# formeo/igaming-platform

Measured on AMD Instinct MI355X. Metric: fraud scores/sec (whole node) + p99 score latency, higher is better.
Workload: dtype fp32

## Files before the change

### csrc/runtime/bindings.cpp

```cpp
#include <pybind11/numpy.h>
#include <pybind11/pybind11.h>
#include <pybind11/stl.h>

#include <atomic>
#include <cstring>
#include <memory>
#include <thread>

#include "account_index.h"
#include "acct_core.h"
#include "acct_devices.h"
#include "audit.h"
#include "h2grpc.h"
#include "cpu_device.h"
#include "cpu_scorer.h"
#include "serve_core.h"
#include "link_index.h"
#include "mult_sketch.h"
#include "executor.h"
#include "onnx_model.h"
#include "sampler.h"
#include "trees.h"
#include "wire.h"
#include "xxh64.h"
// ... 526 lines not shown
        load("ring_ts", c.ring_ts.data(), c.ring_ts.size() * 4);
        load("ring_amt", c.ring_amt.data(), c.ring_amt.size() * 8);
        load("hll", c.hll.data(), c.hll.size());
        load("rt", c.rt.data(), c.rt.size() * sizeof(AcctRT));
        load("batch", c.batch.data(), c.batch.size() * sizeof(AcctBatch));
        load("ext", c.ext.data(), c.ext.size() * 4);
        load("ev", c.ev.data(), c.ev.size() * 2);
      })
      .def_property_readonly("capacity", &CpuScorer::capacity);

  auto view = [](py::array res, py::object feat, py::object ms, wire::ResultView& v,
                 py::array& keep_r, py::object& keep_f, py::object& keep_m) {
    keep_r = py::array_t<uint32_t, py::array::c_style | py::array::forcecast>(res);
    if (keep_r.ndim() != 2 || keep_r.shape(1) != 2) throw std::runtime_error("results must be [n,2] (ResultRec)");
    v.n = size_t(keep_r.shape(0));
    v.res = reinterpret_cast<const ResultRec*>(keep_r.data());
    v.feat = nullptr;
    v.response_ms = nullptr;
    if (!feat.is_none()) {
      auto f = py::array_t<int32_t, py::array::c_style | py::array::forcecast>(feat);
      if (f.ndim() != 2 || f.shape(1) != 32 || size_t(f.shape(0)) != v.n) throw std::runtime_error("features must be [n,32] (FeatRec)");
      keep_f = f;
      v.feat = reinterpret_cast<const FeatRec*>(f.data());
    }
    if (!ms.is_none()) {
      auto t = py::array_t<int64_t, py::array::c_style | py::array::forcecast>(ms);
      if (size_t(t.size()) != v.n) throw std::runtime_error("response_ms length mismatch");
      keep_m = t;
      v.response_ms = t.data();
    }
  };
  m.def("serialize_batch_response", [view](py::array res, py::object feat, py::object ms) {
    wire::ResultView v;
    py::array kr; py::object kf, km;
    view(res, feat, ms, v, kr, kf, km);
    std::string out;
    {
      py::gil_scoped_release rel;
      out = wire::serialize_batch_response(v);
    }
    return py::bytes(out);
  }, py::arg("results"), py::arg("features") = py::none(), py::arg("response_ms") = py::none());
  m.def("serialize_tx_response", [view](py::array res, py::object feat, py::object ms, size_t i) {
    wire::ResultView v;
    py::array kr; py::object kf, km;
    view(res, feat, ms, v, kr, kf, km);
    if (i >= v.n) throw std::runtime_error("index out of range");
    return py::bytes(wire::serialize_tx_response(v, i));
  }, py::arg("results"), py::arg("features") = py::none(), py::arg("response_ms") = py::none(), py::arg("index") = 0);
  m.def("serialize_tx_responses", [view](py::array res, py::object feat, py::object ms) {
    wire::ResultView v;
    py::array kr; py::object kf, km;
    view(res, feat, ms, v, kr, kf, km);
    std::vector<std::string> outs(v.n);
    {
      py::gil_scoped_release rel;
      for (size_t i = 0; i < v.n; ++i) outs[i] = wire::serialize_tx_response(v, i);
    }
    py::list l;
    for (auto& o : outs) l.append(py::bytes(o));
    return l;
  }, py::arg("results"), py::arg("features") = py::none(), py::arg("response_ms") = py::none());
  m.def("serialize_feature_vector", [](py::array feat) {
    auto f = py::array_t<int32_t, py::array::c_style | py::array::forcecast>(feat);
    if (f.size() != 32) throw std::runtime_error("FeatRec must have 32 int32 words");
    return py::bytes(wire::serialize_feature_vector(*reinterpret_cast<const FeatRec*>(f.data())));
  });

  py::class_<StepClock, std::shared_ptr<StepClock>>(m, "StepClock")
      .def(py::init<const std::string&, int, int, bool>(), py::arg("shm_name"), py::arg("world"), py::arg("rank"),
           py::arg("create"))
      .def(py::init<int>(), py::arg("world"))
      .def("issued", &StepClock::issued)
      .def("max_issued", &StepClock::max_issued)
      .def("hold_of", &StepClock::hold_of)
      .def("set_rank", &StepClock::set_rank)
      .def("unlink_shared", &StepClock::unlink_shared)
      .def_property_readonly("world", &StepClock::world)
      .def_property_readonly("rank", &StepClock::rank);

  py::class_<CpuDevice, std::shared_ptr<CpuDevice>>(m, "CpuDevice")
      .def(py::init<std::shared_ptr<CpuScorer>, int, int>(), py::arg("scorer"), py::arg("depth") = 2,
           py::arg("cap") = 8192, py::keep_alive<1, 2>())
      .def("device_ops", [](const CpuDevice& d) { return reinterpret_cast<uintptr_t>(d.ops()); });

  py::class_<ShmXchgDevice, std::shared_ptr<ShmXchgDevice>>(m, "ShmXchgDevice")
      .def(py::init<std::shared_ptr<CpuScorer>, const std::string&, int, int, int, int, bool, double>(),
           py::arg("scorer"), py::arg("shm_name"), py::arg("world"), py::arg("rank"), py::arg("depth"), py::arg("C"),
           py::arg("create"), py::arg("timeout_s") = 60.0, py::keep_alive<1, 2>())
      .def("device_ops", [](const ShmXchgDevice& d) { return reinterpret_cast<uintptr_t>(d.ops()); })
      .def_property_readonly("rows_scored", &ShmXchgDevice::rows_scored)
      .def_property_readonly("slot_violations", &ShmXchgDevice::slot_violations)
      .def_property_readonly("steps", &ShmXchgDevice::steps)
      .def("debug_stall_results_when", &ShmXchgDevice::debug_stall_results_when)
      .def("unlink_shared", &ShmXchgDevice::unlink_shared);

  py::class_<AuditRing, std::shared_ptr<AuditRing>>(m, "AuditRing")
      .def(py::init<int64_t>(), py::arg("capacity"))
      .def("pending", &AuditRing::pending)
      .def("append", [](AuditRing& a, py::array_t<uint32_t, py::array::c_style> res,
                        py::array_t<int32_t, py::array::c_style> slots, int owner, int64_t t_ms, int version) {
        const size_t n = size_t(slots.size());
        if (res.ndim() != 2 || size_t(res.shape(0)) != n || res.shape(1) != 2)
          throw std::runtime_error("AuditRing.append: res must be uint32[n,2] for n slots");
        const ResultRec* r = reinterpret_cast<const ResultRec*>(res.data());
        const int32_t* s = slots.data();
        py::gil_scoped_release rel;
        a.append(r, s, 1, owner, n, t_ms, uint16_t(version));
      }, py::arg("res"), py::arg("slots"), py::arg("owner"), py::arg("t_ms"), py::arg("version"))
      .def_property_readonly("evicted", &AuditRing::evicted)
      .def_property_readonly("appended", &AuditRing::appended)
      .def("flush_sqlite", [](AuditRing& a, const std::string& path, const std::string& schema,
                              std::vector<std::shared_ptr<AccountIndex>> idx) {
        py::gil_scoped_release rel;
        return a.flush_sqlite(path, schema, idx);
      })
      .def_property_readonly("capacity", &AuditRing::capacity)
      .def("flush_segment", [](AuditRing& a, const std::string& dir, const std::string& tag,
                               std::vector<std::shared_ptr<AccountIndex>> idx) {
        py::gil_scoped_release rel;
        return a.flush_segment(dir, tag, idx);
      })
      .def("peek", [](const AuditRing& a, int64_t max) {
        auto v = a.peek(max);
        py::dict d;
        std::vector<int64_t> t(v.size());
        std::vector<int32_t> sl(v.size()), ow(v.size()), ver(v.size());
        std::vector<uint32_t> pk(v.size());
        std::vector<float> ml(v.size());
        for (size_t i = 0; i < v.size(); ++i) {
          t[i] = v[i].t_ms; sl[i] = v[i].slot; ow[i] = v[i].owner; ver[i] = v[i].model_version;
          pk[i] = v[i].packed; ml[i] = v[i].ml;
        }
        d["t_ms"] = vec_np(t); d["slot"] = vec_np(sl); d["owner"] = vec_np(ow); d["model_version"] = vec_np(ver);
        d["packed"] = vec_np(pk); d["ml"] = vec_np(ml);
        return d;
      }, py::arg("max") = 1 << 20);

  m.def("audit_load_segment", [](const std::string& seg, const std::string& db, const std::string& schema) {
    py::gil_scoped_release rel;
    return audit_load_segment(seg, db, schema);
  }, py::arg("segment"), py::arg("db"), py::arg("schema"));

  py::class_<PyGrpc>(m, "GrpcServer")
      .def(py::init([](py::object core, py::function cold, int cold_threads, int batch_threads, py::object acct) {
             auto p = std::make_unique<PyGrpc>();
             std::shared_ptr<ServeCore> c;
             if (!core.is_none()) {
               c = core.cast<PyServe&>().core;
               p->core = core;
             }
             std::shared_ptr<AcctRouter> ar;
             if (!acct.is_none()) {
               ar = acct.cast<PyAcct&>().router;
               p->acct = acct;
             }
             GrpcServer::ColdFn fn = [cb = py::function(cold)](const std::string& path, std::string body) {
               py::gil_scoped_acquire g;
               GrpcReply r;
               try {
                 py::object out = cb(py::str(path), py::bytes(body));
                 if (py::isinstance<py::bytes>(out)) {
                   r.body = out.cast<std::string>();
                 } else {
                   auto t = out.cast<py::tuple>();
                   r.status = t[0].cast<int>();
                   r.message = t[1].cast<std::string>();
// ... 483 lines not shown
```

### csrc/runtime/cpu_device.cpp

```cpp
#include "cpu_device.h"

#include <unistd.h>

#include <chrono>
#include <cstring>
#include <stdexcept>
#include <thread>

namespace igp {
namespace {

void set_err(char* err, int32_t errlen, const char* msg) {
  if (!err || errlen <= 0) return;
  std::strncpy(err, msg, size_t(errlen) - 1);
  err[errlen - 1] = 0;
}

}

CpuDevice::CpuDevice(std::shared_ptr<CpuScorer> sc, int depth, int cap) : sc_(std::move(sc)) {
  if (!sc_ || depth < 1 || cap < 1) throw std::runtime_error("CpuDevice: scorer / depth / capacity");
  slots_.resize(depth);
  for (auto& s : slots_) {
    s.rows.resize(cap);
    s.res.resize(cap);
    s.feat.resize(cap);
  }
  ops_.abi = IGP_DEVICE_OPS_ABI;
  ops_.depth = depth;
  ops_.world = 1;
  ops_.exchange = 0;
  ops_.cap = cap;
  ops_.features_always = 0;
  ops_.ctx = this;
  ops_.rows = &rows_fn;
  ops_.submit = &submit_fn;
  ops_.wait = &wait_fn;
  ops_.results = &results_fn;
  ops_.features = &features_fn;
}

char* CpuDevice::rows_fn(void* ctx, int32_t slot) {
  return reinterpret_cast<char*>(static_cast<CpuDevice*>(ctx)->slots_[slot].rows.data());
}

int32_t CpuDevice::submit_fn(void* ctx, int32_t slot, int32_t n, int32_t, int64_t now, int32_t wf, char* err,
                             int32_t errlen) {
  auto* d = static_cast<CpuDevice*>(ctx);
  Slot& s = d->slots_[slot];
  try {
    s.wf = (wf & IGP_SUBMIT_WANT_FEATURES) != 0;
    d->sc_->score(s.rows.data(), size_t(n), now, true, s.res.data(), s.wf ? s.feat.data() : nullptr);
  } catch (const std::exception& e) {
    set_err(err, errlen, e.what());
    return -1;
  }
  return 0;
}

int32_t CpuDevice::wait_fn(void*, int32_t, int64_t, char*, int32_t) { return 0; }

const void* CpuDevice::results_fn(void* ctx, int32_t slot) {
  return static_cast<CpuDevice*>(ctx)->slots_[slot].res.data();
}

const void* CpuDevice::features_fn(void* ctx, int32_t slot) {
  const Slot& s = static_cast<CpuDevice*>(ctx)->slots_[slot];
  return s.wf ? s.feat.data() : nullptr;
}

ShmXchgDevice::ShmXchgDevice(std::shared_ptr<CpuScorer> sc, const std::string& shm_name, int world, int rank, int depth,
                             int C, bool create, double timeout_s)
    : sc_(std::move(sc)), world_(world), rank_(rank), C_(C), timeout_s_(timeout_s) {
  if (!sc_ || world < 1 || rank < 0 || rank >= world || depth < 1 || C < 1)
    throw std::runtime_error("ShmXchgDevice: bad arguments");
  W_ = sizeof(ResultRec) + sizeof(FeatRec);
  send_bytes_ = size_t(world) * size_t(C + 1) * sizeof(ReqRec);
  res_bytes_ = size_t(world) * size_t(C) * W_;
  const size_t flag_bytes = sizeof(int64_t) * OwnerGenerations::kLineWords * kRing * size_t(world);
  const size_t bytes = sizeof(Counter) * size_t(world) + flag_bytes + size_t(world) * kRing * (send_bytes_ + res_bytes_);
  region_ = Region::shared(shm_name, bytes, create);
  counters_ = reinterpret_cast<Counter*>(region_.base());
  char* flags = reinterpret_cast<char*>(region_.base()) + sizeof(Counter) * size_t(world);
  owners_ = OwnerGenerations(reinterpret_cast<int64_t*>(flags), world, rank);
  data_ = flags + flag_bytes;
  slots_.resize(depth);
  for (auto& s : slots_) {
    s.send.resize(size_t(world) * size_t(C + 1));
    s.recv.resize(res_bytes_);
  }
  compact_.resize(size_t(world) * size_t(C));
  route_.resize(size_t(world) * size_t(C));
  res_.resize(size_t(world) * size_t(C));
  feat_.resize(size_t(world) * size_t(C));
  ops_.abi = IGP_DEVICE_OPS_ABI;
  ops_.depth = depth;
  ops_.world = world;
  ops_.exchange = 1;
  ops_.cap = C;
  ops_.features_always = 1;
  ops_.ctx = this;
  ops_.rows = &rows_fn;
  ops_.submit = &submit_fn;
  ops_.wait = &wait_fn;
  ops_.results = &results_fn;
  ops_.features = &features_fn;
}

ReqRec* ShmXchgDevice::send_area(int r, int q) const {
  return reinterpret_cast<ReqRec*>(data_ + (size_t(r) * kRing + size_t(q)) * send_bytes_);
}

char* ShmXchgDevice::res_area(int r, int q) const {
  return data_ + size_t(world_) * kRing * send_bytes_ + (size_t(r) * kRing + size_t(q)) * res_bytes_;
}

void ShmXchgDevice::wait_all(std::atomic<int64_t> Counter::*field, int64_t target) {
  const auto t_end = std::chrono::steady_clock::now() + std::chrono::duration<double>(timeout_s_);
  for (int spin = 0;; ++spin) {
    bool all = true;
    for (int r = 0; r < world_ && all; ++r) all = (counters_[r].*field).load(std::memory_order_acquire) >= target;
    if (all) return;
    if (spin < 2000) {
      std::this_thread::yield();
    } else {
      if (std::chrono::steady_clock::now() > t_end) throw std::runtime_error("ShmXchgDevice: a peer missed the step");
      std::this_thread::sleep_for(std::chrono::microseconds(20));
    }
  }
}

void ShmXchgDevice::step(int slot, int64_t now) {
// ... 69 lines not shown
```

### csrc/runtime/cpu_device.h

```cpp
#pragma once
#include <atomic>
#include <memory>
#include <string>
#include <vector>

#include "../include/device_ops.h"
#include "../include/records.h"
#include "../include/results_region.h"
#include "cpu_scorer.h"
#include "shm.h"

namespace igp {

class CpuDevice {
 public:
  CpuDevice(std::shared_ptr<CpuScorer> sc, int depth, int cap);
  const IgpDeviceOps* ops() const { return &ops_; }

 private:
  struct Slot {
    std::vector<ReqRec> rows;
    std::vector<ResultRec> res;
    std::vector<FeatRec> feat;
    bool wf = false;
  };
  static char* rows_fn(void* ctx, int32_t slot);
  static int32_t submit_fn(void* ctx, int32_t slot, int32_t n, int32_t seq, int64_t now, int32_t wf, char* err, int32_t errlen);
  static int32_t wait_fn(void* ctx, int32_t slot, int64_t timeout_us, char* err, int32_t errlen);
  static const void* results_fn(void* ctx, int32_t slot);
  static const void* features_fn(void* ctx, int32_t slot);
  std::shared_ptr<CpuScorer> sc_;
  std::vector<Slot> slots_;
  IgpDeviceOps ops_{};
};

class ShmXchgDevice {
 public:
  ShmXchgDevice(std::shared_ptr<CpuScorer> sc, const std::string& shm_name, int world, int rank, int depth, int C,
                bool create, double timeout_s);
  const IgpDeviceOps* ops() const { return &ops_; }
  int64_t rows_scored() const { return rows_scored_.load(); }
  int64_t slot_violations() const { return slot_violations_.load(); }
  int64_t steps() const { return k_; }
  void debug_stall_results_when(const std::string& path) { stall_file_ = path; }
  void unlink_shared() { region_.unlink(); }

 private:
  static constexpr int kRing = 2;
  struct alignas(64) Counter {
    std::atomic<int64_t> posted;
    std::atomic<int64_t> scored;
    std::atomic<int32_t> slot;
    char pad[44];
  };
  struct Slot {
    std::vector<ReqRec> send;
    std::vector<char> recv;
  };
  static char* rows_fn(void* ctx, int32_t slot);
  static int32_t submit_fn(void* ctx, int32_t slot, int32_t n, int32_t seq, int64_t now, int32_t wf, char* err, int32_t errlen);
  static int32_t wait_fn(void* ctx, int32_t slot, int64_t timeout_us, char* err, int32_t errlen);
  static const void* results_fn(void* ctx, int32_t slot);
  static const void* features_fn(void* ctx, int32_t slot);
  void step(int slot, int64_t now);
  void wait_all(std::atomic<int64_t> Counter::*field, int64_t target);
  ReqRec* send_area(int r, int q) const;
  char* res_area(int r, int q) const;

  std::shared_ptr<CpuScorer> sc_;
  Region region_;
  Counter* counters_ = nullptr;
  char* data_ = nullptr;
  int world_, rank_, C_;
  size_t W_, send_bytes_, res_bytes_;
  double timeout_s_;
  int64_t k_ = 0;
  std::string stall_file_;
  bool stalled_ = false;
  OwnerGenerations owners_;
  std::vector<Slot> slots_;
  std::vector<ReqRec> compact_;
  std::vector<int32_t> route_;
  std::vector<ResultRec> res_;
  std::vector<FeatRec> feat_;
  std::atomic<int64_t> rows_scored_{0};
  std::atomic<int64_t> slot_violations_{0};
  IgpDeviceOps ops_{};
};

}
```

### csrc/runtime/serve_core.cpp

```cpp
#include "serve_core.h"
#include "mult_sketch.h"
#include "thread_name.h"

#include <algorithm>
#include <chrono>
#include <cstring>
#include <ctime>
#include <stdexcept>

namespace igp {

StepClock::StepClock(const std::string& shm_name, int world, int rank, bool create) : world_(world), rank_(rank) {
  if (world < 1 || rank < 0 || rank >= world) throw std::runtime_error("StepClock: rank / world");
  region_ = Region::shared(shm_name, sizeof(Slot) * size_t(world), create);
  slots_ = reinterpret_cast<Slot*>(region_.base());
}

StepClock::StepClock(int world) : world_(world) {
  if (world < 1) throw std::runtime_error("StepClock: world");
  region_ = Region::anon(sizeof(Slot) * size_t(world));
  slots_ = reinterpret_cast<Slot*>(region_.base());
}

void StepClock::post(int64_t issued) { slots_[rank_].issued.store(issued, std::memory_order_release); }
int64_t StepClock::issued(int r) const { return slots_[r].issued.load(std::memory_order_acquire); }
int64_t StepClock::max_issued() const {
  int64_t m = 0;
  for (int r = 0; r < world_; ++r) m = std::max(m, issued(r));
  return m;
}
void StepClock::hold(int64_t gen) { slots_[rank_].hold.store(gen, std::memory_order_release); }
int64_t StepClock::hold_of(int r) const { return slots_[r].hold.load(std::memory_order_acquire); }
bool StepClock::all_hold(int64_t gen) const {
  for (int r = 0; r < world_; ++r)
    if (hold_of(r) < gen) return false;
  return true;
}

struct ServeCore::Item {
  int kind = 0;
  size_t n = 0;
  std::vector<ReqRec> rows;
  std::vector<int32_t> perm;
  std::vector<int32_t> ostart;
  std::vector<int32_t> ocur;
  int64_t remaining = 0;
  int64_t taken = 0;
  int64_t aborted_rows = 0;
  int64_t now = 0;
  bool wf = false;
  MultSketch mult;
  ResultRec* res = nullptr;
  FeatRec* feat = nullptr;
  ResultRec res1{};
  FeatRec feat1{};
  uint64_t tag = 0;
  int64_t t0 = 0, t_enq = 0;
  int64_t t_issue = 0;
  int32_t seq_first = 0, seq_last = 0;
  std::mutex m;
  std::condition_variable cv;
  std::vector<std::pair<Step*, Seg>> ready;
  bool failed = false;
  std::string err;
};

int64_t ServeCore::now_ns() {
  return std::chrono::duration_cast<std::chrono::nanoseconds>(std::chrono::steady_clock::now().time_since_epoch())
      .count();
}

namespace {
int64_t wall_s() { return int64_t(std::time(nullptr)); }
constexpr size_t kResBytes = sizeof(ResultRec), kFeatBytes = sizeof(FeatRec);
}

ServeCore::ServeCore(std::vector<std::shared_ptr<AccountIndex>> indexes, const IgpDeviceOps* dev, int rank,
                     std::shared_ptr<StepClock> clock, Options opt)
    : idx_(std::move(indexes)), dev_(dev), rank_(rank), clock_(std::move(clock)), opt_(opt) {
  if (!dev_ || dev_->abi != IGP_DEVICE_OPS_ABI) throw std::runtime_error("ServeCore: device function table ABI mismatch");
  world_ = dev_->world;
  exchange_ = dev_->exchange != 0;
  cap_ = dev_->cap;
  depth_ = dev_->depth;
  if ((int)idx_.size() != world_) throw std::runtime_error("ServeCore: one account index per owner expected");
  if (cap_ < 1 || depth_ < 1) throw std::runtime_error("ServeCore: device capacity / depth");
  if (exchange_ && !clock_) throw std::runtime_error("ServeCore: the exchange needs a StepClock");
  if (exchange_ && clock_->world() != world_) throw std::runtime_error("ServeCore: StepClock world");
  if (!exchange_ && world_ != 1) throw std::runtime_error("ServeCore: a direct device serves one owner");
  for (auto& a : dec_) a.store(0);
  for (auto& a : act_) a.store(0);
  steps_.resize(depth_);
  for (int s = 0; s < depth_; ++s) {
    steps_[s] = std::make_unique<Step>();
    free_slots_.push_back(depth_ - 1 - s);
  }
  if (clock_) issued_.store(clock_->issued(rank_));
  seq_ = opt_.seq0;
  threads_.emplace_back([this] {
    name_thread("core-step");
    stepper_loop();
  });
  threads_.emplace_back([this] {
    name_thread("core-done");
    completion_loop();
  });
  for (int i = 0; i < std::max(1, opt_.finishers); ++i)
    threads_.emplace_back([this] {
      name_thread("core-fin");
      finisher_loop();
    });
  threads_.emplace_back([this] {
    name_thread("core-link");
    link_loop();
  });
}

ServeCore::~ServeCore() {
  try {
    stop();
  } catch (...) {
  }
}

void ServeCore::resolve_rows(std::vector<wire::TxRow>& rows, Item* it) {
  const size_t n = rows.size();
  const int32_t enc = it->wf ? FV_ENC_BIT : 0;
  it->n = n;
  it->rows.resize(n);
  thread_local std::vector<std::string_view> ids;
  thread_local std::vector<uint64_t> hs;
  thread_local std::vector<int32_t> slots;
  ids.resize(n);
  hs.resize(n);
  slots.resize(n);
  if (world_ == 1) {
    for (size_t k = 0; k < n; ++k) {
      ids[k] = rows[k].account;
      hs[k] = rows[k].account_hash;
// ... 2 lines not shown
    for (size_t k = 0; k < n; ++k) {
      it->rows[k] = rows[k].rec;
      it->rows[k].slot = slots[k];
      it->rows[k].tx_type |= enc;
    }
    it->ocur.assign(1, 0);
    it->ostart = {0, int32_t(n)};
    if (!exchange_) it->mult.build(it->rows.data(), n);
  } else {
    it->ostart.assign(world_ + 1, 0);
    thread_local std::vector<int32_t> own;
    own.resize(n);
    for (size_t k = 0; k < n; ++k) {
      own[k] = int32_t(rows[k].account_hash % uint64_t(world_));
      ++it->ostart[own[k] + 1];
    }
    for (int o = 0; o < world_; ++o) it->ostart[o + 1] += it->ostart[o];
    it->ocur.assign(it->ostart.begin(), it->ostart.end() - 1);
    std::vector<int32_t> fill(it->ostart.begin(), it->ostart.end() - 1);
    it->perm.resize(n);
    for (size_t k = 0; k < n; ++k) {
      const int32_t pos = fill[own[k]]++;
      it->perm[pos] = int32_t(k);
      ids[pos] = rows[k].account;
      hs[pos] = rows[k].account_hash;
    }
    for (int o = 0; o < world_; ++o) {
      const int32_t b = it->ostart[o], e = it->ostart[o + 1];
      if (e > b) idx_[o]->lookup_views(ids.data() + b, hs.data() + b, size_t(e - b), true, slots.data() + b, nullptr);
    }
    for (size_t pos = 0; pos < n; ++pos) {
      it->rows[pos] = rows[it->perm[pos]].rec;
      it->rows[pos].slot = slots[pos];
      it->rows[pos].tx_type |= enc;
    }
  }
  bool link_room = false;
  if (links_ && n) {
    std::lock_guard<std::mutex> g(l_mu_);
    link_room = lq_.size() < kLinkQueue;
  }
  if (link_room) {
    std::vector<uint64_t> d(n);
    std::vector<int64_t> a(n);
    for (size_t pos = 0; pos < n; ++pos) {
      const int32_t o = world_ == 1 ? 0 : int32_t(rows[it->perm[pos]].account_hash % uint64_t(world_));
      d[pos] = it->rows[pos].dev_hash;
      a[pos] = it->rows[pos].slot >= 0 ? ((int64_t(o) << 32) | it->rows[pos].slot) : -1;
    }
    std::lock_guard<std::mutex> g(l_mu_);
    if (lq_.size() < kLinkQueue) {
      links_->note_queued();
      lq_.emplace_back(std::move(d), std::move(a));
      l_cv_.notify_one();
    }
  }
}

void ServeCore::enqueue(Item* it) {
  it->remaining = int64_t(it->n);
  it->t_enq = now_ns();
  {
    std::lock_guard<std::mutex> lk(q_mu_);
    if (stopping_ || stopped_) throw std::runtime_error("ServeCore: stopped");
    queue_.push_back(it);
    queued_rows_ += int64_t(it->n);
  }
  q_cv_.notify_all();
}

void ServeCore::wait_item(Item* it) {
  size_t done = 0;
  std::unique_lock<std::mutex> l(it->m);
  while (done + size_t(it->aborted_rows) < it->n) {
    it->cv.wait(l, [&] { return !it->ready.empty() || done + size_t(it->aborted_rows) >= it->n; });
    std::vector<std::pair<Step*, Seg>> batch;
    batch.swap(it->ready);
    l.unlock();
    const int64_t t = now_ns();
    for (auto& [st, seg] : batch) {
      if (st->failed) {
        it->failed = true;
        if (it->err.empty()) it->err = st->err;
      } else {
        finish_seg(*st, seg);
      }
      done += size_t(seg.count);
      release_step_ref(st);
    }
    a_copy_.fetch_add(now_ns() - t, std::memory_order_relaxed);
    l.lock();
  }
}

std::string ServeCore::score_batch(const char* data, size_t n, int64_t now, int64_t t0_ns) {
  const std::string_view v = score_batch_view(data, n, now, t0_ns);
  return std::string(v.data(), v.size());
}

std::string_view ServeCore::score_batch_view(const char* data, size_t n, int64_t now, int64_t t0_ns) {
  const int64_t t0 = t0_ns > 0 ? t0_ns : now_ns();
  thread_local std::vector<wire::TxRow> rows;
  rows.clear();
  const int64_t ta = now_ns();
  wire::parse_batch_rows(data, n, rows);
  const int64_t tb = now_ns();
  if (rows.empty()) return {};
  Item it;
  thread_local std::vector<ReqRec> rows_buf;
  thread_local std::vector<uint16_t> mult_buf;
  it.rows.swap(rows_buf);
  it.mult.c.swap(mult_buf);
  struct GiveBack {
    std::vector<ReqRec>& buf;
    std::vector<uint16_t>& mbuf;
    Item& item;
    ~GiveBack() {
      buf.swap(item.rows);
      mbuf.swap(item.mult.c);
    }
  } give_back{rows_buf, mult_buf, it};
  it.kind = 0;
  it.now = now >= 0 ? now : wall_s();
  it.wf = opt_.features;
  resolve_rows(rows, &it);
  const int64_t tc = now_ns();
  thread_local std::vector<ResultRec> res;
  thread_local std::vector<FeatRec> feat;
  res.resize(it.n);
  if (it.wf) feat.resize(it.n);
  it.res = res.data();
  it.feat = it.wf ? feat.data() : nullptr;
  enqueue(&it);
  const int64_t tq = it.t_enq;
  wait_item(&it);
  if (it.failed) throw std::runtime_error("ServeCore: batch failed: " + it.err);
  const int64_t td = now_ns();
  const std::string_view out = wire::batch_response_scratch(it.res, it.feat, nullptr, (td - t0) / 1000000, it.n);
  const int64_t te = now_ns();
  CallTimings& ct = last_timings_tl();
  ct = CallTimings{tb - ta, tc - tb, it.t_issue - tq, td - it.t_issue, te - td, te - t0, int64_t(it.n), it.seq_first,
                   it.seq_last};
  a_parse_.fetch_add(tb - ta, std::memory_order_relaxed);
  a_resolve_.fetch_add(tc - tb, std::memory_order_relaxed);
  a_serialize_.fetch_add(te - td, std::memory_order_relaxed);
  a_items_.fetch_add(1, std::memory_order_relaxed);
  a_rows_.fetch_add(int64_t(it.n), std::memory_order_relaxed);
  return out;
}

void ServeCore::score_rows(const ReqRec* rows, const int32_t* owners, size_t n, int64_t now, bool want_features,
                           ResultRec* res, FeatRec* feat) {
  if (n == 0) return;
  Item it;
  it.kind = 0;
  it.n = n;
  it.now = now >= 0 ? now : wall_s();
  it.wf = want_features && feat != nullptr;
  it.res = res;
  it.feat = it.wf ? feat : nullptr;
  if (world_ == 1) {
    it.rows.assign(rows, rows + n);
    it.ocur.assign(1, 0);
    it.ostart = {0, int32_t(n)};
    if (!exchange_) it.mult.build(it.rows.data(), n);
  } else {
    if (!owners) throw std::runtime_error("ServeCore.score_rows: owners required when world > 1");
    it.ostart.assign(world_ + 1, 0);
    for (size_t k = 0; k < n; ++k) {
      if (owners[k] < 0 || owners[k] >= world_) throw std::runtime_error("ServeCore.score_rows: owner out of range");
      ++it.ostart[owners[k] + 1];
    }
    for (int o = 0; o < world_; ++o) it.ostart[o + 1] += it.ostart[o];
    it.ocur.assign(it.ostart.begin(), it.ostart.end() - 1);
    std::vector<int32_t> fill(it.ocur);
    it.perm.resize(n);
    it.rows.resize(n);
    for (size_t k = 0; k < n; ++k) {
      const int32_t pos = fill[owners[k]]++;
      it.perm[pos] = int32_t(k);
      it.rows[pos] = rows[k];
    }
  }
  enqueue(&it);
  wait_item(&it);
  if (it.failed) throw std::runtime_error("ServeCore: batch failed: " + it.err);
}

void ServeCore::submit_tx(const char* data, size_t n, uint64_t tag, int64_t now, int64_t t0_ns) {
  auto* it = new Item();
  it->kind = 1;
  it->tag = tag;
  it->t0 = t0_ns > 0 ? t0_ns : now_ns();
  it->now = now >= 0 ? now : wall_s();
  it->wf = opt_.features;
  it->res = &it->res1;
  it->feat = it->wf ? &it->feat1 : nullptr;
  try {
    std::vector<wire::TxRow> rows(1);
    wire::parse_tx_row(data, n, rows[0]);
    resolve_rows(rows, it);
    enqueue(it);
  } catch (const std::exception& e) {
    std::vector<Done> d;
    d.push_back(Done{tag, std::string(), e.what()});
    delete it;
    deliver(std::move(d));
  }
}

void ServeCore::submit_tx_many(const TxCall* calls, size_t n, int64_t now) {
  if (n == 0) return;
  thread_local std::vector<wire::TxRow> rows;
  thread_local std::vector<Item*> items;
  thread_local std::vector<std::string_view> ids;
  thread_local std::vector<uint64_t> hs;
  thread_local std::vector<int32_t> slots;
  thread_local std::vector<uint8_t> ok;
  rows.resize(n);
  items.assign(n, nullptr);
  ok.assign(n, 0);
  std::vector<Done> bad;
  const int64_t wnow = now >= 0 ? now : wall_s();
  const int32_t enc = opt_.features ? FV_ENC_BIT : 0;
  for (size_t k = 0; k < n; ++k) {
    try {
      wire::parse_tx_row(calls[k].data, calls[k].n, rows[k]);
      ok[k] = 1;
    } catch (const std::exception& e) {
      bad.push_back(Done{calls[k].tag, std::string(), e.what()});
    }
// ... 661 lines not shown
```

### csrc/runtime/serve_core.h

```cpp
#pragma once
#include <atomic>
#include <functional>
#include <condition_variable>
#include <cstdint>
#include <deque>
#include <memory>
#include <mutex>
#include <string>
#include <thread>
#include <vector>

#include "../include/device_ops.h"
#include "../include/records.h"
#include "account_index.h"
#include "audit.h"
#include "link_index.h"
#include "shm.h"
#include "wire.h"

namespace igp {

inline constexpr const char* kColdPrefix = "cold: ";

class StepClock {
 public:
  StepClock(const std::string& shm_name, int world, int rank, bool create);
  explicit StepClock(int world);
  int world() const { return world_; }
  int rank() const { return rank_; }
  void set_rank(int r) { rank_ = r; }
  void post(int64_t issued);
  int64_t issued(int r) const;
  int64_t max_issued() const;
  void hold(int64_t gen);
  bool all_hold(int64_t gen) const;
  int64_t hold_of(int r) const;
  void unlink_shared() { region_.unlink(); }

 private:
  struct alignas(64) Slot {
    std::atomic<int64_t> issued;
    std::atomic<int64_t> hold;
    char pad[48];
  };
  Region region_;
  Slot* slots_ = nullptr;
  int world_ = 1, rank_ = 0;
};

struct CallTimings {
  int64_t parse = 0, resolve = 0, queue = 0, device = 0, serialize = 0, total = 0, rows = 0;
  int32_t seq_first = 0, seq_last = 0;
};
inline CallTimings& last_timings_tl() {
  thread_local CallTimings t;
  return t;
}

struct ServeStats {
  int64_t items = 0, rows = 0, steps = 0, empty_steps = 0, unary = 0;
  int64_t parse_ns = 0, resolve_ns = 0, pack_ns = 0, device_ns = 0, copy_ns = 0, serialize_ns = 0, queue_ns = 0;
  int64_t submit_ns = 0, wait_errors = 0, max_step_rows = 0;
  int64_t release_ns = 0, slot_wait_ns = 0, rows_wait_ns = 0, slot_waits = 0, slot_wait_inflight = 0;
  int64_t actions[4] = {0, 0, 0, 0};
  int64_t deciles[11] = {0};
  int64_t ml_high = 0, blacklisted = 0, scored = 0;
};

class ServeCore {
 public:
  struct Options {
    int max_wait_us = 200;
    int64_t timeout_us = -1;
    int finishers = 2;
    bool features = true;
    int64_t stop_timeout_us = 30000000;
    int32_t seq0 = 0;
    int unary_depth = 0;
  };
  static constexpr int64_t kUnaryWindowNs = 20000000;

  ServeCore(std::vector<std::shared_ptr<AccountIndex>> indexes, const IgpDeviceOps* dev, int rank,
            std::shared_ptr<StepClock> clock, Options opt);
  ~ServeCore();
  ServeCore(const ServeCore&) = delete;
  ServeCore& operator=(const ServeCore&) = delete;

  std::string score_batch(const char* data, size_t n, int64_t now, int64_t t0_ns);
  std::string_view score_batch_view(const char* data, size_t n, int64_t now, int64_t t0_ns);
  void score_rows(const ReqRec* rows, const int32_t* owners, size_t n, int64_t now, bool want_features,
                  ResultRec* res, FeatRec* feat);
  void submit_tx(const char* data, size_t n, uint64_t tag, int64_t now, int64_t t0_ns);
  struct TxCall {
    const char* data;
    size_t n;
    uint64_t tag;
    int64_t t0_ns;
  };
  void submit_tx_many(const TxCall* calls, size_t n, int64_t now);
  struct Done {
    uint64_t tag;
    std::string bytes;
    std::string err;
  };
  size_t poll(std::vector<Done>& out, size_t max, int64_t timeout_us);
  using Sink = std::function<void(std::vector<Done>&&)>;
  static constexpr uint64_t kSinkTag = uint64_t(1) << 63;
  void set_sink(Sink sink) {
    std::lock_guard<std::mutex> g(out_mu_);
    sink_ = std::move(sink);
  }

  void pause();
  void resume();
  void set_device(const IgpDeviceOps* dev);
  void stop();
  void abort();

  void set_links(std::shared_ptr<LinkIndex> links) { links_ = std::move(links); }
  void set_audit(std::shared_ptr<AuditRing> ring) { audit_ = std::move(ring); }
  void set_model_version(int v) { model_ver_.store(uint16_t(v)); }
  ServeStats stats(bool reset);
  int64_t issued() const { return issued_.load(); }
  int32_t seq() const { return seq_; }
  int late_steps() const { return late_.load(); }
  int world() const { return world_; }
  int pending_items();

  static int64_t now_ns();

 private:
  struct Item;
  struct Seg {
    Item* item;
    int32_t owner;
    int32_t item_pos;
    int32_t dev_pos;
    int32_t count;
  };
  struct Step {
    int slot = 0;
    int32_t seq = 0;
    int n = 0;
    bool wf = false;
    int64_t t_submit = 0, t_done = 0;
    std::vector<Seg> segs;
    std::atomic<int> refs{0};
    bool failed = false;
    std::string err;
  };

  void stepper_loop();
  void note_wait(int64_t ServeStats::*field, int64_t ns);
  void completion_loop();
  void finisher_loop();
  void deliver(std::vector<Done>&& outs);
  void link_loop();
  void enqueue(Item* it);
  void wait_item(Item* it);
  bool issue_step(std::unique_lock<std::mutex>& lk, bool allow_empty);
  int next_slot_locked() const;
  void finish_seg(const Step& st, const Seg& s);
  void release_step_ref(Step* st);
  void resolve_rows(std::vector<wire::TxRow>& rows, Item* it);
  void converge(int64_t gen);
  void record_decisions(const ResultRec* r, int n);
  void audit_seg(const ResultRec* r, const ReqRec* rows, int owner, int n);

  std::vector<std::shared_ptr<AccountIndex>> idx_;
  const IgpDeviceOps* dev_;
  int world_, rank_;
  bool exchange_;
  int cap_, depth_;
  std::shared_ptr<StepClock> clock_;
  Options opt_;
  std::shared_ptr<LinkIndex> links_;
  std::shared_ptr<AuditRing> audit_;
  Sink sink_;
  std::atomic<uint16_t> model_ver_{1};

  std::mutex q_mu_;
  std::condition_variable q_cv_;
  std::deque<Item*> queue_;
  std::deque<Item*> uqueue_;
  int64_t queued_rows_ = 0;
  std::vector<int> free_slots_;
  std::vector<std::unique_ptr<Step>> steps_;
  int inflight_ = 0;
  int64_t last_unary_ns_ = 0;
  bool stopping_ = false, stopped_ = false, paused_ = false, pause_req_ = false, aborting_ = false;
  int64_t hold_gen_ = 0;
  bool held_ = false;
  std::condition_variable idle_cv_;

  std::mutex c_mu_;
  std::condition_variable c_cv_;
  std::deque<Step*> done_fifo_;
  bool c_stop_ = false;

  std::mutex f_mu_;
  std::condition_variable f_cv_;
  struct FTask {
    Step* step;
    std::vector<Seg> segs;
  };
  std::deque<FTask> ftasks_;
  bool f_stop_ = false;
  std::mutex out_mu_;
  std::condition_variable out_cv_;
  std::deque<Done> outq_;

  std::mutex l_mu_;
  std::condition_variable l_cv_;
  static constexpr size_t kLinkQueue = 4;
  std::deque<std::pair<std::vector<uint64_t>, std::vector<int64_t>>> lq_;
  bool l_stop_ = false;

  std::atomic<int64_t> issued_{0};
  std::atomic<int> late_{0};
  int32_t seq_ = 0;
  int64_t gen_ = 0;

  std::mutex st_mu_;
  ServeStats st_;
  std::atomic<int64_t> a_parse_{0}, a_resolve_{0}, a_serialize_{0}, a_copy_{0}, a_items_{0}, a_rows_{0};
  std::atomic<int64_t> dec_[11], act_[4], hi_{0}, bl_{0}, scored_{0};

  std::vector<std::thread> threads_;
};

}
```

### csrc/runtime/wire.cpp

```cpp
#include "wire.h"

#include <cstring>

#include "pb.h"
#include "xxh64.h"

namespace igp::wire {

const char* const kReasonCodes[12] = {
    "HIGH_VELOCITY", "NEW_ACCOUNT_LARGE_TX", "MULTIPLE_DEVICES", "IP_COUNTRY_MISMATCH",
    "VPN_DETECTED", "RAPID_DEPOSIT_WITHDRAW", "BONUS_ABUSE", "KNOWN_FRAUDSTER",
    "ML_HIGH_RISK", "SUSPICIOUS_PATTERN", "MULTI_ACCOUNT", "DEVICE_FINGERPRINT_MISMATCH"};

void RequestBatch::clear() {
  account_id.clear(); account_hash.clear(); amount.clear(); tx_type.clear();
  device_hash.clear(); fp_hash.clear(); ip_hash.clear(); arena.clear();
}

void RequestBatch::reserve(size_t n) {
  account_id.reserve(n); account_hash.reserve(n); amount.reserve(n); tx_type.reserve(n);
  device_hash.reserve(n); fp_hash.reserve(n); ip_hash.reserve(n);
}

const std::string& RequestBatch::own(const char* data, size_t n) {
// ... 242 lines not shown
  o.i32(T1(3, 0), 1, x.tx_count_1h);
  o.i64(T1(4, 0), 1, x.tx_sum_1h);
  o.f32(T1(5, 5), 1, x.tx_avg_1h);
  o.i32(T1(6, 0), 1, x.unique_devices_24h);
  o.i32(T1(7, 0), 1, x.unique_ips_24h);
  o.i32(T1(8, 0), 1, x.ip_country_changes_7d);
  o.i32(T1(9, 0), 1, x.device_age_days);
  o.i32(T1(10, 0), 1, x.account_age_days);
  o.i64(T1(11, 0), 1, x.total_deposits);
  o.i64(T1(12, 0), 1, x.total_withdrawals);
  o.i64(T1(13, 0), 1, x.net_deposit);
  o.i32(T1(14, 0), 1, x.deposit_count);
  o.i32(T1(15, 0), 1, x.withdraw_count);
  o.i32(T2(16, 0), 2, x.time_since_last_tx);
  o.i32(T2(17, 0), 2, x.session_duration);
  o.f32(T2(18, 5), 2, x.avg_bet_size);
  o.f32(T2(19, 5), 2, x.win_rate);
  o.boolean(T2(20, 0), 2, x.flags & FR_VPN);
  o.boolean(T2(21, 0), 2, x.flags & FR_PROXY);
  o.boolean(T2(22, 0), 2, x.flags & FR_TOR);
  o.boolean(T2(23, 0), 2, x.flags & FR_DISPOSABLE);
  o.i32(T2(24, 0), 2, x.bonus_claim_count);
  o.f32(T2(25, 5), 2, x.bonus_wager_rate);
  o.boolean(T2(26, 0), 2, x.flags & FR_BONUS_ONLY);
}

inline char* close_len(char* slot, char* end) {
  const size_t n = size_t(end - slot - 1);
  if (__builtin_expect(n < 128, 1)) {
    *slot = char(n);
    return end;
  }
  char lb[10];
  Out lo{lb};
  lo.varint(n);
  const size_t ln = size_t(lo.p - lb);
  std::memmove(slot + ln, slot + 1, n);
  std::memcpy(slot, lb, ln);
  return slot + ln + n;
}

inline char* write_tx_body(char* out, const ResultRec& r, const FeatRec* f, int64_t ms) {
  FastOut o{out};
  const uint32_t p = r.packed;
  o.uvar(T1(1, 0), 1, IGP_RES_SCORE(p));
  o.uvar(T1(2, 0), 1, IGP_RES_ACTION(p));
  uint32_t reasons = IGP_RES_REASONS(p);
  if (reasons) {
    const ReasonTable& t = reasons_table();
    while (reasons) {
      const int b = __builtin_ctz(reasons);
      std::memcpy(o.p, t.enc[b], 32);
      o.p += t.len[b];
      reasons &= reasons - 1;
    }
  }
  o.uvar(T1(4, 0), 1, IGP_RES_RULE(p));
  o.f32(T1(5, 5), 1, r.ml);
  o.i64(T1(6, 0), 1, ms);
  if (f) {
    *o.p = char(T1(7, pb::LEN));
    const uint8_t img = reinterpret_cast<const uint8_t*>(f)[sizeof(FeatRec) - 1];
    if (img & FV_IMG_ENCODED) {
      const size_t len = img & 0x7f;
      o.p[1] = char(len);
      std::memcpy(o.p + 2, f, 128);
      o.p += 2 + len;
    } else {
      char* slot = o.p + 1;
      o.p = slot + 1;
      write_feature_vector(o, *f);
      o.p = close_len(slot, o.p);
    }
  }
  return o.p;
}

}

size_t write_tx_response(char* out, const ResultRec& r, const FeatRec* f, int64_t ms) {
  return size_t(write_tx_body(out, r, f, ms) - out);
}

size_t write_batch_response(char* dst, const ResultRec* r, const FeatRec* f, const int64_t* ms, int64_t ms_all,
                            size_t n) {
  char* p = dst;
  for (size_t i = 0; i < n; ++i) {
    *p = char(T1(1, pb::LEN));
    char* slot = p + 1;
    p = close_len(slot, write_tx_body(slot + 1, r[i], f ? f + i : nullptr, ms ? ms[i] : ms_all));
  }
  return size_t(p - dst);
}

std::string_view batch_response_scratch(const ResultRec* r, const FeatRec* f, const int64_t* ms, int64_t ms_all,
                                        size_t n) {
  thread_local std::unique_ptr<char[]> scratch;
  thread_local size_t scratch_cap = 0;
  const size_t need = n * kMaxBatchRowBytes;
  if (scratch_cap < need) {
    scratch.reset(new char[need]);
    scratch_cap = need;
  }
  return std::string_view(scratch.get(), write_batch_response(scratch.get(), r, f, ms, ms_all, n));
}

void append_batch_response(std::string& out, const ResultRec* r, const FeatRec* f, const int64_t* ms, int64_t ms_all,
                           size_t n) {
  const std::string_view v = batch_response_scratch(r, f, ms, ms_all, n);
  out.append(v.data(), v.size());
}

std::string serialize_feature_vector(const FeatRec& x) {
  char body[400];
  FastOut o{body};
  write_feature_vector(o, x);
  return std::string(body, size_t(o.p - body));
}

std::string serialize_tx_response(const ResultView& v, size_t i) {
  char body[kMaxTxResponse];
  const size_t n = write_tx_response(body, v.res[i], v.feat ? v.feat + i : nullptr, v.response_ms ? v.response_ms[i] : 0);
  return std::string(body, n);
}

std::string serialize_batch_response(const ResultView& v) {
  std::string out;
  append_batch_response(out, v.res, v.feat, v.response_ms, 0, v.n);
  return out;
}

}
```

### csrc/runtime/wire.h

```cpp
#pragma once
#include <cstdint>
#include <memory>
#include <string>
#include <string_view>
#include <vector>

#include "../include/records.h"

namespace igp::wire {

struct RequestBatch {
  std::vector<std::string_view> account_id;
  std::vector<uint64_t> account_hash;
  std::vector<int64_t> amount;
  std::vector<uint8_t> tx_type;
  std::vector<uint64_t> device_hash, fp_hash, ip_hash;
  std::vector<std::unique_ptr<std::string>> arena;
  size_t size() const { return amount.size(); }
  void clear();
  void reserve(size_t n);
  const std::string& own(const char* data, size_t n);
};

struct TxRow {
  std::string_view account;
  uint64_t account_hash;
  ReqRec rec;
};

uint8_t tx_type_id(const char* s, size_t n);

void parse_tx(const char* data, size_t n, RequestBatch& out);
void parse_batch(const char* data, size_t n, RequestBatch& out);
void parse_tx_row(const char* data, size_t n, TxRow& out);
void parse_batch_rows(const char* data, size_t n, std::vector<TxRow>& out);

extern const char* const kReasonCodes[12];

struct ResultView {
  const ResultRec* res;
  const FeatRec* feat;
  const int64_t* response_ms;
  size_t n;
};
std::string serialize_tx_response(const ResultView& v, size_t i);
std::string serialize_batch_response(const ResultView& v);
std::string serialize_feature_vector(const FeatRec& f);

constexpr size_t kMaxTxResponse = 1024;
size_t write_tx_response(char* out, const ResultRec& r, const FeatRec* f, int64_t ms);
constexpr size_t kMaxBatchRowBytes = kMaxTxResponse + 8;
size_t write_batch_response(char* dst, const ResultRec* r, const FeatRec* f, const int64_t* ms, int64_t ms_all,
                            size_t n);
std::string_view batch_response_scratch(const ResultRec* r, const FeatRec* f, const int64_t* ms, int64_t ms_all,
                                        size_t n);
void append_batch_response(std::string& out, const ResultRec* r, const FeatRec* f, const int64_t* ms, int64_t ms_all,
                           size_t n);

}
```

Measured before the change: 129.8 million.

## Stream batch responses per segment straight into the output buffer

For non-exchange devices, batch scoring now serialises each completed segment directly into a caller-supplied response buffer as the step finishes, instead of copying results into per-thread arrays and serialising after the whole batch completes. This removes the intermediate result/feature copy and overlaps serialisation with other steps still in flight. It also adds a score_batch_into API with an allocator callback and a CpuDevice fault-injection hook that adds atomic loads on the submit path. Segments must now arrive in row order or the batch fails, and the per-response latency stamp is taken per segment rather than once at the end.

```diff
diff --git a/csrc/runtime/bindings.cpp b/csrc/runtime/bindings.cpp
--- a/csrc/runtime/bindings.cpp
+++ b/csrc/runtime/bindings.cpp
@@ -632,7 +632,8 @@
   py::class_<CpuDevice, std::shared_ptr<CpuDevice>>(m, "CpuDevice")
       .def(py::init<std::shared_ptr<CpuScorer>, int, int>(), py::arg("scorer"), py::arg("depth") = 2,
            py::arg("cap") = 8192, py::keep_alive<1, 2>())
-      .def("device_ops", [](const CpuDevice& d) { return reinterpret_cast<uintptr_t>(d.ops()); });
+      .def("device_ops", [](const CpuDevice& d) { return reinterpret_cast<uintptr_t>(d.ops()); })
+      .def("debug_fail_steps", &CpuDevice::debug_fail_steps, py::arg("n"), py::arg("after") = 0);
 
   py::class_<ShmXchgDevice, std::shared_ptr<ShmXchgDevice>>(m, "ShmXchgDevice")
       .def(py::init<std::shared_ptr<CpuScorer>, const std::string&, int, int, int, int, bool, double>(),
diff --git a/csrc/runtime/cpu_device.cpp b/csrc/runtime/cpu_device.cpp
--- a/csrc/runtime/cpu_device.cpp
+++ b/csrc/runtime/cpu_device.cpp
@@ -48,6 +48,10 @@
                              int32_t errlen) {
   auto* d = static_cast<CpuDevice*>(ctx);
   Slot& s = d->slots_[slot];
+  if (d->fail_steps_.load() > 0 && d->pass_steps_.fetch_sub(1) <= 0 && d->fail_steps_.fetch_sub(1) > 0) {
+    set_err(err, errlen, "CpuDevice: injected step failure");
+    return -1;
+  }
   try {
     s.wf = (wf & IGP_SUBMIT_WANT_FEATURES) != 0;
     d->sc_->score(s.rows.data(), size_t(n), now, true, s.res.data(), s.wf ? s.feat.data() : nullptr);
diff --git a/csrc/runtime/cpu_device.h b/csrc/runtime/cpu_device.h
--- a/csrc/runtime/cpu_device.h
+++ b/csrc/runtime/cpu_device.h
@@ -16,6 +16,10 @@
  public:
   CpuDevice(std::shared_ptr<CpuScorer> sc, int depth, int cap);
   const IgpDeviceOps* ops() const { return &ops_; }
+  void debug_fail_steps(int n, int after) {
+    pass_steps_.store(after);
+    fail_steps_.store(n);
+  }
 
  private:
   struct Slot {
@@ -31,6 +35,7 @@
   static const void* features_fn(void* ctx, int32_t slot);
   std::shared_ptr<CpuScorer> sc_;
   std::vector<Slot> slots_;
+  std::atomic<int> fail_steps_{0}, pass_steps_{0};
   IgpDeviceOps ops_{};
 };
 
diff --git a/csrc/runtime/serve_core.cpp b/csrc/runtime/serve_core.cpp
--- a/csrc/runtime/serve_core.cpp
+++ b/csrc/runtime/serve_core.cpp
@@ -55,6 +55,10 @@
   ResultRec res1{};
   FeatRec feat1{};
   uint64_t tag = 0;
+  bool stream = false;
+  char* out_cur = nullptr;
+  size_t ser_rows = 0;
+  int64_t ser_ns = 0;
   int64_t t0 = 0, t_enq = 0;
   int64_t t_issue = 0;
   int32_t seq_first = 0, seq_last = 0;
@@ -223,15 +227,41 @@
       if (st->failed) {
         it->failed = true;
         if (it->err.empty()) it->err = st->err;
-      } else {
+      } else if (!it->stream) {
         finish_seg(*st, seg);
+      } else if (!it->failed) {
+        stream_seg(*st, seg);
       }
       done += size_t(seg.count);
       release_step_ref(st);
     }
-    a_copy_.fetch_add(now_ns() - t, std::memory_order_relaxed);
+    const int64_t dt = now_ns() - t;
+    if (it->stream) {
+      it->ser_ns += dt;
+      a_serialize_.fetch_add(dt, std::memory_order_relaxed);
+    } else {
+      a_copy_.fetch_add(dt, std::memory_order_relaxed);
+    }
     l.lock();
   }
+}
+
+void ServeCore::stream_seg(const Step& st, const Seg& s) {
+  Item* it = s.item;
+  if (size_t(s.item_pos) != it->ser_rows) {
+    it->failed = true;
+    if (it->err.empty())
+      it->err = "segment out of row order: rows from " + std::to_string(s.item_pos) + " after " +
+                std::to_string(it->ser_rows) + " serialised";
+    return;
+  }
+  const ResultRec* r = static_cast<const ResultRec*>(dev_->results(dev_->ctx, st.slot)) + s.dev_pos;
+  const FeatRec* f = it->wf ? static_cast<const FeatRec*>(dev_->features(dev_->ctx, st.slot)) : nullptr;
+  it->out_cur = wire::write_batch_rows(it->out_cur, r, f ? f + s.dev_pos : nullptr, (now_ns() - it->t0) / 1000000,
+                                       size_t(s.count));
+  it->ser_rows += size_t(s.count);
+  record_decisions(r, s.count);
+  audit_seg(r, it->rows.data() + s.item_pos, 0, s.count);
 }
 
 std::string ServeCore::score_batch(const char* data, size_t n, int64_t now, int64_t t0_ns) {
@@ -240,13 +270,13 @@
 }
 
 std::string_view ServeCore::score_batch_view(const char* data, size_t n, int64_t now, int64_t t0_ns) {
+  char* buf = nullptr;
+  const size_t len = score_batch_into(data, n, now, t0_ns, [&](size_t ub) { return buf = wire::response_scratch(ub); });
+  return len ? std::string_view(buf, len) : std::string_view();
+}
+
+size_t ServeCore::score_batch_into(const char* data, size_t n, int64_t now, int64_t t0_ns, const Alloc& alloc) {
   const int64_t t0 = t0_ns > 0 ? t0_ns : now_ns();
-  thread_local std::vector<wire::TxRow> rows;
-  rows.clear();
-  const int64_t ta = now_ns();
-  wire::parse_batch_rows(data, n, rows);
-  const int64_t tb = now_ns();
-  if (rows.empty()) return {};
   Item it;
   thread_local std::vector<ReqRec> rows_buf;
   thread_local std::vector<uint16_t> mult_buf;
@@ -264,30 +294,52 @@
   it.kind = 0;
   it.now = now >= 0 ? now : wall_s();
   it.wf = opt_.features;
+  it.t0 = t0;
+  thread_local std::vector<wire::TxRow> rows;
+  rows.clear();
+  const int64_t ta = now_ns();
+  wire::parse_batch_rows(data, n, rows);
+  const int64_t tb = now_ns();
+  if (rows.empty()) return 0;
   resolve_rows(rows, &it);
   const int64_t tc = now_ns();
+  char* const out = alloc(it.n * wire::kMaxBatchRowBytes);
+  if (!out) throw std::runtime_error("ServeCore: no response buffer");
   thread_local std::vector<ResultRec> res;
   thread_local std::vector<FeatRec> feat;
-  res.resize(it.n);
-  if (it.wf) feat.resize(it.n);
-  it.res = res.data();
-  it.feat = it.wf ? feat.data() : nullptr;
+  if (!exchange_) {
+    it.stream = true;
+    it.out_cur = out;
+  } else {
+    res.resize(it.n);
+    if (it.wf) feat.resize(it.n);
+    it.res = res.data();
+    it.feat = it.wf ? feat.data() : nullptr;
+  }
   enqueue(&it);
   const int64_t tq = it.t_enq;
   wait_item(&it);
   if (it.failed) throw std::runtime_error("ServeCore: batch failed: " + it.err);
   const int64_t td = now_ns();
-  const std::string_view out = wire::batch_response_scratch(it.res, it.feat, nullptr, (td - t0) / 1000000, it.n);
+  size_t len;
+  int64_t ser = it.ser_ns;
+  if (it.stream) {
+    if (it.ser_rows != it.n) throw std::runtime_error("ServeCore: batch failed: rows missing from the response");
+    len = size_t(it.out_cur - out);
+  } else {
+    len = wire::write_batch_response(out, it.res, it.feat, nullptr, (td - t0) / 1000000, it.n);
+    ser = now_ns() - td;
+    a_serialize_.fetch_add(ser, std::memory_order_relaxed);
+  }
   const int64_t te = now_ns();
   CallTimings& ct = last_timings_tl();
-  ct = CallTimings{tb - ta, tc - tb, it.t_issue - tq, td - it.t_issue, te - td, te - t0, int64_t(it.n), it.seq_first,
-                   it.seq_last};
+  ct = CallTimings{tb - ta, tc - tb, it.t_issue - tq, td - it.t_issue - it.ser_ns, ser, te - t0, int64_t(it.n),
+                   it.seq_first, it.seq_last};
   a_parse_.fetch_add(tb - ta, std::memory_order_relaxed);
   a_resolve_.fetch_add(tc - tb, std::memory_order_relaxed);
-  a_serialize_.fetch_add(te - td, std::memory_order_relaxed);
   a_items_.fetch_add(1, std::memory_order_relaxed);
   a_rows_.fetch_add(int64_t(it.n), std::memory_order_relaxed);
-  return out;
+  return len;
 }
 
 void ServeCore::score_rows(const ReqRec* rows, const int32_t* owners, size_t n, int64_t now, bool want_features,
diff --git a/csrc/runtime/serve_core.h b/csrc/runtime/serve_core.h
--- a/csrc/runtime/serve_core.h
+++ b/csrc/runtime/serve_core.h
@@ -88,6 +88,8 @@
 
   std::string score_batch(const char* data, size_t n, int64_t now, int64_t t0_ns);
   std::string_view score_batch_view(const char* data, size_t n, int64_t now, int64_t t0_ns);
+  using Alloc = std::function<char*(size_t)>;
+  size_t score_batch_into(const char* data, size_t n, int64_t now, int64_t t0_ns, const Alloc& alloc);
   void score_rows(const ReqRec* rows, const int32_t* owners, size_t n, int64_t now, bool want_features,
                   ResultRec* res, FeatRec* feat);
   void submit_tx(const char* data, size_t n, uint64_t tag, int64_t now, int64_t t0_ns);
@@ -161,6 +163,7 @@
   bool issue_step(std::unique_lock<std::mutex>& lk, bool allow_empty);
   int next_slot_locked() const;
   void finish_seg(const Step& st, const Seg& s);
+  void stream_seg(const Step& st, const Seg& s);
   void release_step_ref(Step* st);
   void resolve_rows(std::vector<wire::TxRow>& rows, Item* it);
   void converge(int64_t gen);
diff --git a/csrc/runtime/wire.cpp b/csrc/runtime/wire.cpp
--- a/csrc/runtime/wire.cpp
+++ b/csrc/runtime/wire.cpp
@@ -348,27 +348,38 @@
   return size_t(write_tx_body(out, r, f, ms) - out);
 }
 
-size_t write_batch_response(char* dst, const ResultRec* r, const FeatRec* f, const int64_t* ms, int64_t ms_all,
-                            size_t n) {
+char* write_batch_rows(char* dst, const ResultRec* r, const FeatRec* f, int64_t ms, size_t n) {
   char* p = dst;
   for (size_t i = 0; i < n; ++i) {
     *p = char(T1(1, pb::LEN));
     char* slot = p + 1;
-    p = close_len(slot, write_tx_body(slot + 1, r[i], f ? f + i : nullptr, ms ? ms[i] : ms_all));
-  }
+    p = close_len(slot, write_tx_body(slot + 1, r[i], f ? f + i : nullptr, ms));
+  }
+  return p;
+}
+
+size_t write_batch_response(char* dst, const ResultRec* r, const FeatRec* f, const int64_t* ms, int64_t ms_all,
+                            size_t n) {
+  if (!ms) return size_t(write_batch_rows(dst, r, f, ms_all, n) - dst);
+  char* p = dst;
+  for (size_t i = 0; i < n; ++i) p = write_batch_rows(p, r + i, f ? f + i : nullptr, ms[i], 1);
   return size_t(p - dst);
 }
 
-std::string_view batch_response_scratch(const ResultRec* r, const FeatRec* f, const int64_t* ms, int64_t ms_all,
-                                        size_t n) {
+char* response_scratch(size_t need) {
   thread_local std::unique_ptr<char[]> scratch;
   thread_local size_t scratch_cap = 0;
-  const size_t need = n * kMaxBatchRowBytes;
   if (scratch_cap < need) {
     scratch.reset(new char[need]);
     scratch_cap = need;
   }
-  return std::string_view(scratch.get(), write_batch_response(scratch.get(), r, f, ms, ms_all, n));
+  return scratch.get();
+}
+
+std::string_view batch_response_scratch(const ResultRec* r, const FeatRec* f, const int64_t* ms, int64_t ms_all,
+                                        size_t n) {
+  char* buf = response_scratch(n * kMaxBatchRowBytes);
+  return std::string_view(buf, write_batch_response(buf, r, f, ms, ms_all, n));
 }
 
 void append_batch_response(std::string& out, const ResultRec* r, const FeatRec* f, const int64_t* ms, int64_t ms_all,
diff --git a/csrc/runtime/wire.h b/csrc/runtime/wire.h
--- a/csrc/runtime/wire.h
+++ b/csrc/runtime/wire.h
@@ -50,6 +50,8 @@
 constexpr size_t kMaxTxResponse = 1024;
 size_t write_tx_response(char* out, const ResultRec& r, const FeatRec* f, int64_t ms);
 constexpr size_t kMaxBatchRowBytes = kMaxTxResponse + 8;
+char* write_batch_rows(char* dst, const ResultRec* r, const FeatRec* f, int64_t ms, size_t n);
+char* response_scratch(size_t need);
 size_t write_batch_response(char* dst, const ResultRec* r, const FeatRec* f, const int64_t* ms, int64_t ms_all,
                             size_t n);
 std::string_view batch_response_scratch(const ResultRec* r, const FeatRec* f, const int64_t* ms, int64_t ms_all,
```

New measurement: 138.5 million, median of 6. +6.7%, better.
